# delehef/asgart

Hardware: AMD Instinct MI355X
Metric: Mbp/s probe+extend (direct+RC, k=20 g=100) (higher is better)
Workload: dtype u64 keys / u32 SA

## Files before the change

asgart_amd/csrc/device_base.hpp:

```cpp
#pragma once

#include "search_dev.hpp"

#include <type_traits>

namespace asgart {

constexpr int kTiers = 7;
constexpr int kRunsStat = kTiers + 1;

enum Counter {
    CT_BIG = 0,
    CT_SEG,
    CT_SCAN_TICKET,
    CT_FAM,
    CT_SD,
    CT_OVF,
    CT_TOTAL_HITS,
    CT_N_SKIPPED,
    CT_CARD_SKIPPED,
    CT_WITH_HITS,
    CT_RAW_HITS,
    CT_SEARCHED,
    CT_BISECT,
    CT_OVF_CURSOR,
    CT_AMBIG,
    CT_RANOUT,
    CT_EARLY_N = 34,
    CT_EARLY_CUR = 36,
    CT_RANK = 38,
    CT_BIG0 = 39,
    CT_ALG_BYTES = 68,
    CT_FLT_REJECTED,
    CT_LONGSEG,
    CT_ALG_BYTES16,
    CT_HIST_PEAK = 72,
    CT_HIST_PROBES = 88,
    CT_N1 = 104,
    CT_NF = 111,
    CT_CUR1 = 112,
    CT_CURF = 119,
    CT_OVF1 = 120,
    CT_BUSY1 = 128,
    CT_WGS1 = 136,
    CT_TPROBES1 = 144,
    CT_THITS1 = 152,
    CT_SEGMAX1 = 160,
    CT_CLUSTER_BARREN = 168,
    CT_CLUSTER_CUR = 169,
    CT_COUNT = 176
};

__device__ inline int chunk_of(const ChunkTable &ch, uint32_t g) {
    int lo = 0, hi = ch.n_chunks;
    while (hi - lo > 1) {
        int mid = (lo + hi) >> 1;
        if (ch.pbase[mid] <= g) lo = mid; else hi = mid;
    }
    return lo;
}

__device__ inline int chunk_of_uniform(const ChunkTable &ch, uint32_t g) {
    g = __builtin_amdgcn_readfirstlane(g);
    int lo = 0, hi = ch.n_chunks;
    while (hi - lo > 1) {
        const int mid = __builtin_amdgcn_readfirstlane((lo + hi) >> 1);
        if (ch.pbase[mid] <= g) lo = mid; else hi = mid;
    }
    return __builtin_amdgcn_readfirstlane(lo);
}

__device__ inline bool keep_hit(uint64_t x, uint64_t i, uint64_t s, uint64_t L, bool reverse) {
    if (!reverse) return x > i + s;
    return x != i && x >= s + L - i;
}

__device__ inline void lds_barrier() { __asm__ volatile("s_waitcnt lgkmcnt(0)\n\ts_barrier" ::: "memory"); }

__device__ inline uint32_t uni(uint32_t v) { return (uint32_t)__builtin_amdgcn_readfirstlane((int)v); }
__device__ inline unsigned long long uni(unsigned long long v) {
    return ((unsigned long long)uni((uint32_t)(v >> 32)) << 32) | uni((uint32_t)v);
}
__device__ inline uint32_t lane_of(uint32_t v, uint32_t l) {
    return (uint32_t)__builtin_amdgcn_readlane((int)v, (int)l);
}
__device__ inline unsigned long long lane_of(unsigned long long v, uint32_t l) {
    return ((unsigned long long)lane_of((uint32_t)(v >> 32), l) << 32) | lane_of((uint32_t)v, l);
}

__device__ inline uint32_t wave_incl_scan(uint32_t x) {
#define ASGART_DPP_ADD(ctrl, rows) \
    x += (uint32_t)__builtin_amdgcn_update_dpp(0, (int)x, ctrl, rows, 0xf, false)
    ASGART_DPP_ADD(0x111, 0xf);
    ASGART_DPP_ADD(0x112, 0xf);
    ASGART_DPP_ADD(0x114, 0xf);
    ASGART_DPP_ADD(0x118, 0xf);
    ASGART_DPP_ADD(0x142, 0xa);
    ASGART_DPP_ADD(0x143, 0xc);
#undef ASGART_DPP_ADD
    return x;
}

// ... 15 lines not shown
```

asgart_amd/csrc/extend_common_dev.hpp:

```cpp
#pragma once

#include "device_base.hpp"

namespace asgart {

constexpr uint32_t kTombstone = 0xFFFFFFFFu;

#ifdef ASGART_PROFILE_EXTEND
#define PROF_DECL unsigned long long pf_t0 = 0, pf_acc[12] = {0, 0, 0, 0, 0, 0, 0, 0, 0, 0, 0, 0}
#define PROF_START() pf_t0 = __builtin_amdgcn_s_memtime()
#define PROF_STOP(slot) pf_acc[slot] += __builtin_amdgcn_s_memtime() - pf_t0
#define PROF_COUNT(slot, v) pf_acc[slot] += (v)
#define PROF_MAX(slot, v) pf_acc[slot] = pf_acc[slot] > (unsigned long long)(v) ? pf_acc[slot] : (unsigned long long)(v)
#define PROF_SEG_BEGIN() const unsigned long long pf_seg0 = __builtin_amdgcn_s_memtime()
#define PROF_FLUSH()                                                             \
    do {                                                                         \
        const unsigned long long pf_dt = __builtin_amdgcn_s_memtime() - pf_seg0; \
        if (lane == 0 && atomicMax(&P.ctr[28], pf_dt) < pf_dt) {                 \
            P.ctr[29] = g0;                                                      \
            P.ctr[30] = ((unsigned long long)pf_acc[5] << 32) | pf_acc[3];       \
            P.ctr[31] = ((unsigned long long)pf_acc[10] << 32) | pf_acc[11];     \
            P.ctr[32] = pf_acc[0];                                               \
            P.ctr[33] = pf_acc[6];                                               \
            P.ctr[25] = pf_acc[9];                                               \
// ... 22 lines not shown
#define PROF_MAX(slot, v)
#define PROF_SEG_BEGIN()
#define PROF_FLUSH()
#endif
constexpr int kHitBatch = 1024;
constexpr uint32_t kNoSeq = 0xFFFFFFFFu;

struct RangeRun {
    uint32_t g_begin, g_stop;
    uint32_t g_seg0;
    uint32_t emit_from;
    uint32_t flags;
    uint32_t split;
    uint32_t pad0, pad1;
};
constexpr uint32_t kRunNoEmit = 1u;
constexpr uint32_t kRunLast = 2u;
constexpr uint32_t kRunDumpCap = 5120;
template <class PosT> constexpr uint32_t kDumpWords = sizeof(PosT) == 4 ? 8u : 12u;
struct SplitSeg {
    uint32_t g_seg0, run_base, n_ranges, cut_base;
    uint32_t span, hits, tier, warm;
};

template <class PosT>
struct ExtParams {
    const RangeRun *runs;
    uint32_t *run_meta, *run_dump;
    RunParams rp;
    const uint32_t *p_filt;
    const unsigned long long *row_off;
    const PosT *hits;
    const uint32_t *seg_list;
    const unsigned long long *n_seg_ptr;
    unsigned long long *cursor;
    SdRec *recs;
    unsigned long long rec_cap;
    uint32_t *ovf_list;
    unsigned long long *ovf_count;
    char *scratch;
    uint32_t gen_bits;
    uint32_t escalate_cost;
    uint32_t cap_limit;
    uint32_t heavy_cap;
    uint32_t solo_hits;
    uint32_t k8_delay;
    uint32_t tier;
    unsigned long long *seg_slots;
    unsigned long long *ctr;
    unsigned long long *hb;
};

template <class PosT>
__device__ inline void heartbeat(const ExtParams<PosT> &P, uint32_t g0, uint32_t at) {
    if (P.hb) {
        unsigned long long *slot = P.hb + 2u * (blockIdx.x % 256u);
        __builtin_nontemporal_store((unsigned long long)g0 | 1ull << 63, slot);
        __builtin_nontemporal_store((unsigned long long)at, slot + 1);
    }
}

template <class PosT>
__device__ inline bool arm_accepts(PosT x, PosT re, uint32_t thr, uint32_t k) {
    const PosT lo = (PosT)(re - k + 1u);
    const uint64_t w = thr ? (uint64_t)thr + k - 1u : 0u;
    return (uint64_t)(PosT)(x - lo) < w;
}

__device__ inline uint32_t arm_threshold(uint64_t left_len, uint32_t G) {
    const uint64_t tenth = left_len <= 0xFFFFFFFFull ? (uint64_t)((uint32_t)left_len / 10u) : left_len / 10u;
    const uint64_t thr = tenth > (uint64_t)G ? tenth : (uint64_t)G;
    return thr > 0xFFFFFFFFull ? 0xFFFFFFFFu : (uint32_t)thr;
}

constexpr uint32_t kRecChunk = 32;
constexpr uint32_t kVoidStart = 0xFFFFFFFFu;
struct RecAlloc {
    unsigned long long next = 0;
    uint32_t left = 0;
};
template <class PosT>
__device__ inline void wg_begin(const ExtParams<PosT> &P) {
    if (threadIdx.x == 0 && P.tier >= 1u && P.tier <= (uint32_t)kRunsStat) {
        atomicAdd(&P.ctr[CT_BUSY1 + P.tier - 1u], 0ull - wall_clock64());
    }
}
template <class PosT>
__device__ inline void seg_clock(const ExtParams<PosT> &P, bool last = false) {
    if (!P.seg_slots || P.tier < 2u || P.tier > (uint32_t)kRunsStat) return;
    const unsigned long long now = wall_clock64();
    const unsigned long long prev = atomicExch(&P.seg_slots[blockIdx.x & 4095u], last ? 0ull : now);
    if (prev && now > prev) atomicMax(&P.ctr[CT_SEGMAX1 + P.tier - 1u], now - prev);
}
template <class PosT>
__device__ inline void wg_busy(const ExtParams<PosT> &P) {
    if (threadIdx.x == 0 && P.tier >= 1u && P.tier <= (uint32_t)kRunsStat) {
        seg_clock(P, true);
        atomicAdd(&P.ctr[CT_BUSY1 + P.tier - 1u], wall_clock64());
        atomicAdd(&P.ctr[CT_WGS1 + P.tier - 1u], 1ull);
    }
}
template <class PosT>
__device__ inline void rec_flush(RecAlloc &ra, const ExtParams<PosT> &P, int lane) {
    if ((uint32_t)lane < ra.left && ra.next + (unsigned)lane < P.rec_cap) P.recs[ra.next + (unsigned)lane].g_start = kVoidStart;
    ra.left = 0;
}
template <class PosT>
__device__ inline unsigned long long rec_slot(RecAlloc &ra, const ExtParams<PosT> &P, unsigned long long em, int lane) {
    const uint32_t n = (uint32_t)__popcll(em);
    if (n > ra.left) {
        rec_flush(ra, P, lane);
        const uint32_t take = n > kRecChunk ? n : kRecChunk;
        unsigned long long b = 0;
        if (lane == 0) b = atomicAdd(&P.ctr[CT_SD], (unsigned long long)take);
        ra.next = lane_of(b, 0u);
        ra.left = take;
    }
    const unsigned long long at = ra.next + (unsigned)__popcll(em & ((1ull << lane) - 1ull));
    ra.next += n;
    ra.left -= n;
    return at;
}

struct SegHeader {
    uint64_t cs, cl;
    bool rev;
    uint32_t pb;
    uint32_t chunk_end;
    uint32_t g_end;
};
__device__ inline SegHeader load_segment(const RunParams &rp, uint32_t g0) {
    const int c = chunk_of_uniform(rp.ch, g0);
    SegHeader s;
    s.cs = rp.ch.start[c];
    s.cl = rp.ch.len[c];
    s.rev = (rp.mode_of(c) & 2u) != 0u;
    s.pb = rp.ch.pbase[c];
    s.chunk_end = rp.ch.pbase[c + 1];
    s.g_end = min(s.chunk_end, rp.win_end(g0));
    return s;
}

struct ProbeBatch {
    uint32_t f_l, rel_l;
    unsigned long long base;
    uint32_t n;
    uint32_t tot;
    unsigned long long hm, qm;
};
template <int HB>
// ... 73 lines not shown
```

asgart_amd/csrc/extend_k8_dev.hpp:

```cpp
#pragma once

#include "extend_fast_dev.hpp"

namespace asgart {

#ifdef ASGART_PROFILE_EXTEND
#define K7T_DECL unsigned long long k7t[4] = {0, 0, 0, 0}, k7t0 = 0, k7n = 0
#define K7T_MARK() k7t0 = __builtin_amdgcn_s_memtime()
#define K7T_LAP(j)                                                   \
    do {                                                             \
        const unsigned long long k7now = __builtin_amdgcn_s_memtime(); \
        k7t[j] += k7now - k7t0;                                      \
        k7t0 = k7now;                                                \
    } while (0)
#define K7T_STEP() ++k7n
#define K7C(slot, v) do { if (wave == 0u && lane == 0) atomicAdd(&P.ctr[slot], (unsigned long long)(v)); } while (0)
#define K7U_DECL unsigned long long k7u[8] = {0, 0, 0, 0, 0, 0, 0, 0}, k7u0 = 0
#define K7U_MARK() k7u0 = __builtin_amdgcn_s_memtime()
#define K7U_LAP(j)                                                   \
    do {                                                             \
        const unsigned long long k7now = __builtin_amdgcn_s_memtime(); \
        k7u[j] += k7now - k7u0;                                      \
        k7u0 = k7now;                                                \
    } while (0)
#define K7U_FLUSH()                                                                       \
    do {                                                                                  \
        if (lane == 0)                                                                    \
            for (int k7j = 0; k7j < 8; ++k7j) atomicAdd(&P.ctr[57 + k7j], k7u[k7j]);       \
        for (int k7j = 0; k7j < 8; ++k7j) k7u[k7j] = 0;                                   \
    } while (0)
#define K7T_FLUSH(cls)                                                                      \
    do {                                                                                    \
        if (lane == 0)                                                                      \
            for (int k7j = 0; k7j < 4; ++k7j) atomicAdd(&P.ctr[40 + 4 * (cls) + k7j], k7t[k7j]); \
        if (lane == 0 && (cls) == 0) atomicAdd(&P.ctr[52], k7n);                            \
        k7t[0] = k7t[1] = k7t[2] = k7t[3] = 0;                                              \
        k7n = 0;                                                                            \
    } while (0)
#else
#define K7T_DECL
#define K7T_MARK()
#define K7T_LAP(j)
#define K7T_STEP()
#define K7C(slot, v)
#define K7U_DECL
#define K7U_MARK()
#define K7U_LAP(j)
#define K7U_FLUSH()
#define K7T_FLUSH(cls)
#endif

#define K7_RARE(x) __builtin_expect(!!(x), 0)
#define K7_USUAL(x) __builtin_expect(!!(x), 1)

constexpr uint32_t K7_PREV = 1u;
constexpr uint32_t K7_CUR = 2u;
constexpr uint32_t K7_LATE = 4u;
constexpr uint32_t K7_LAST = 8u;
constexpr uint32_t K7_GIVEUP = 16u;
constexpr uint32_t K7_OVF = 1u;
constexpr uint32_t K7_STAGE = 2u;
constexpr uint32_t K7_CLEAR = 4u;


constexpr uint32_t K8_CLEARNOW = 32u;
constexpr uint32_t K8_OVF = 1u;
constexpr uint32_t K8_STILL = 2u;
constexpr uint32_t K8_BIG = 4u;

template <class PosT, int S, int NT, int HB, int kRows = 1024, int kE = 2, bool RANGE = false>
__global__ __launch_bounds__(NT) void extend_k8_kernel(ExtParams<PosT> P) {
    constexpr int NW = NT / 64, NWA = NW - 2;
    constexpr int CAP = S * NWA * 64;
    constexpr int NE = S * NWA;
    constexpr uint32_t kRowsWalk = 62;
    constexpr uint32_t kBitWords = (uint32_t)kRows / 32u;
    using Tab = ArmTable<PosT>;
    using WinT = typename Tab::WinT;
    constexpr bool kWidePos = Tab::kWidePos;
    constexpr uint32_t kTabBytes = (uint32_t)(kRows * kE * 8);
    constexpr uint32_t kCmdWords = 32;
    constexpr uint32_t kNewMax = kWidePos ? (uint32_t)HB / 2u : (uint32_t)HB;
    static_assert(!RANGE || S * NWA * 64 <= (int)kRunDumpCap, "runs over ranges: dump capacity");
    static_assert(NW >= 4 && HB <= 1024 && S <= 8 && NE <= 128 && (kRows & (kRows - 1)) == 0 && kE == 2 && kRows <= 2048 && CAP < 65536,
                  "shape");
    if (NT >= 1024) __builtin_amdgcn_s_setprio(3);

    __shared__ __attribute__((aligned(16))) unsigned long long s_tab[2][kRows * kE];
    __shared__ PosT s_hits[3 * HB];
    __shared__ __attribute__((aligned(16))) uint32_t s_best[3][HB];
    __shared__ unsigned long long s_stash[3][kStash];
    __shared__ uint32_t s_rowbits[3][kRows / 32];
    __shared__ __attribute__((aligned(16))) uint32_t s_pull[2][8];
    __shared__ uint32_t s_slot[2][NWA][8];
    __shared__ __attribute__((aligned(16))) uint32_t s_nstash[4];
#ifdef K8_SINGLE_FREE
    constexpr uint32_t kFreeBufs = 1;
#else
    constexpr uint32_t kFreeBufs = 2;
#endif
    __shared__ __attribute__((aligned(16))) uint32_t s_free[kFreeBufs][NWA][8];
    __shared__ PosT s_newx[2][kNewMax];
    __shared__ uint32_t s_newch[2][kNewMax];
    __shared__ uint16_t s_newh[2][RANGE ? kNewMax : 1u];
    __shared__ __attribute__((aligned(16))) uint32_t s_cmd[3][kCmdWords];
    __shared__ __attribute__((aligned(16))) uint32_t s_mid[8];
    __shared__ PosT s_cle[CAP], s_crs[CAP];
    __shared__ unsigned long long s_seg[3];
    __shared__ uint32_t s_end[4];
    __shared__ unsigned long long s_bcast;
    __shared__ uint32_t s_sink[64];
    __shared__ uint32_t s_never;

    const int tid = threadIdx.x, lane = tid & 63;
    const uint32_t wave = (uint32_t)__builtin_amdgcn_readfirstlane(tid >> 6);
    const bool is_rank = wave == (uint32_t)NWA, is_plan = wave == (uint32_t)(NWA + 1);
    const unsigned long long lt_mask = (1ull << lane) - 1ull;
    RecAlloc rec_alloc;
    wg_begin(P);
    K7T_DECL;
    K7U_DECL;
#ifdef ASGART_PROFILE_EXTEND
    unsigned long long k7_sum_a = 0, k7_sum_cnt = 0, k7_sum_n = 0;
#endif

    PosT a_ls[S], a_re[S];
    uint32_t a_thr[S], a_gap[S], a_seq[S], c_h[S];
#pragma unroll
    for (int L = 0; L < S; ++L) {
        a_seq[L] = kNoSeq;
        a_ls[L] = a_re[L] = 0;
        a_thr[L] = a_gap[L] = 0;
        c_h[L] = 0;
    }
    uint32_t livemask = 0;
    uint32_t gen = 0, par = 0, tri = 0;
    auto clear_table = [&]() {
        for (uint32_t e = tid; e < (uint32_t)(2 * kRows * kE); e += NT) (&s_tab[0][0])[e] = 0ull;
    };
    clear_table();
    if (tid == 0) s_never = kNever;
    lds_barrier();

    char *const tab0 = reinterpret_cast<char *>(&s_tab[0][0]);
    char *const best0 = reinterpret_cast<char *>(&s_best[0][0]);

    for (;;) {
        if (tid == 0) s_bcast = atomicAdd(P.cursor, 1ull);
        if (tid < 4) s_nstash[tid] = 0u;
        if (tid < 16) (&s_pull[0][0])[tid] = 0u;
        for (uint32_t j = tid; j < 3u * kBitWords; j += NT) (&s_rowbits[0][0])[j] = 0u;
        for (uint32_t j = tid; j < kFreeBufs * (uint32_t)(NWA * 8); j += NT) (&s_free[0][0][0])[j] = 64u;
        for (uint32_t j = tid; j < (uint32_t)(2 * NWA * 8); j += NT) (&s_slot[0][0][0])[j] = 0u;
        lds_barrier();
        const unsigned long long seg = uni(s_bcast);
        lds_barrier();
        if (seg >= *P.n_seg_ptr) break;
        RangeRun run{};
        uint32_t emit_from_i = 0;
        if constexpr (RANGE) {
            run = P.runs[seg];
            run.g_begin = uni(run.g_begin);
            run.g_stop = uni(run.g_stop);
            run.g_seg0 = uni(run.g_seg0);
            run.emit_from = uni(run.emit_from);
// ... 701 lines not shown
                atomicAdd(&P.ctr[26], k7_sum_a);
                atomicAdd(&P.ctr[27], k7_sum_cnt);
                atomicAdd(&P.ctr[21], k7_sum_n);
                const unsigned long long k7_dt = __builtin_amdgcn_s_memtime() - k7_seg0;
                if (atomicMax(&P.ctr[28], k7_dt) < k7_dt) {
                    P.ctr[29] = g0;
                    P.ctr[30] = k7_sum_n << 32;
                    P.ctr[31] = (k7_sum_a << 32) | (k7_sum_cnt & 0xffffffffull);
                }
            }
            k7_sum_a = k7_sum_cnt = k7_sum_n = 0;
#endif
            if (!overflow) {
                const uint32_t (*const fr)[8] = s_free[sp & (kFreeBufs - 1u)];
                const uint32_t fv = lane < NE ? fr[lane % NWA][lane / NWA] : 0u;
                uint32_t total_free = lane_of(wave_incl_scan(fv), 63u);
                if constexpr (NE > 64) {
                    const uint32_t fv2 = lane + 64 < NE ? fr[(lane + 64) % NWA][(lane + 64) / NWA] : 0u;
                    total_free += lane_of(wave_incl_scan(fv2), 63u);
                }
                const bool ran_out = uni(s_end[1]) != 0u;
                if constexpr (RANGE) {
                    if (lane == 0) {
                        uint32_t *m = P.run_meta + seg * 16ull;
                        m[1] = fam_seq;
                        m[2] = fam_open ? 1u : 0u;
                        m[3] = 0u;
                        m[5] = (uint32_t)wall_clock64() - s_end[3];
                    }
                }
                if (fam_open && total_free == (uint32_t)CAP) fam_open = false;
                if (RANGE && !(run.flags & kRunLast)) {
                } else if (ran_out) {
                    if (lane == 0) atomicAdd(&P.ctr[CT_RANOUT], 1ull);
                } else if (fam_open) {
                    emit_records(lane == 0, (PosT)0, (PosT)0, (PosT)0, (PosT)0, kTombstone, fam_seq);
                }
            } else if (lane == 0) {
                if constexpr (RANGE) {
                    P.run_meta[seg * 16ull + 4ull] = 1u;
                } else {
                    const unsigned long long at = atomicAdd(P.ovf_count, 1ull);
                    if (P.ovf_list) P.ovf_list[at] = g0;
                }
            }
        } else {
            const RunParams &rp = P.rp;
            const uint32_t k = (uint32_t)rp.k, step = (uint32_t)rp.step, G = rp.G;
            const uint32_t thr0 = arm_threshold(k, G);
            const uint32_t bsh = bucket_shift(G, k);
            const uint32_t kGenBits = min(Tab::kGenMax, max(2u, P.gen_bits));
            const uint32_t g0 = RANGE ? run.g_seg0 : P.seg_list[seg];
            if (lane == 0) {
                heartbeat(P, g0, 0u);
                seg_clock(P);
            }
            const SegHeader sg = load_segment(rp, g0);
            const uint32_t g_end = RANGE ? min(sg.g_end, run.g_stop) : sg.g_end;
            if (lane == 0) {
                if constexpr (RANGE) s_end[3] = (uint32_t)wall_clock64();
                s_seg[0] = g0;
                s_seg[1] = sg.cs;
                s_seg[2] = sg.cl | ((unsigned long long)sg.rev << 63);
            }
            uint32_t quiet = 0, pend = 0;
            bool done = false, giveup = false;
            uint32_t hbuf = 2;
            uint32_t g = RANGE ? run.g_begin : g0, pos = 0;
            ProbeBatch bt{};
            bool staged = false;
            auto open_batch = [&]() {
                if (lane == 0) heartbeat(P, g0, g);
                bt = load_batch<HB>(P.p_filt, P.row_off, g, g_end, lane);
                pos = 0;
                staged = false;
                return bt.n != 0u;
            };
            struct Probe {
                uint32_t cnt, off, tb, bb, g10, pend;
                uint64_t i;
            };
            struct Plan {
                uint32_t flags, pre;
                unsigned long long st_base;
                uint32_t st_tot, st_buf;
                Probe q;
            };
            const Probe no_probe{0, 0, 0, 0, 0, 0, 0};
            bool opened = false;
            auto next_probe = [&](Probe &nx) -> bool {
                for (;;) {
                    uint32_t q;
                    const uint32_t b = next_hit(bt, pos, q);
                    if (q) {
                        quiet += q;
                        pend += q * step;
                        if (quiet >= rp.tstar) {
                            done = true;
                            return false;
                        }
                    }
                    if (b < 64u) {
                        quiet = 0;
                        pos = b + 1;
                        opened = false;
                        if (!staged) {
                            hbuf = hbuf == 2u ? 0u : hbuf + 1u;
                            opened = true;
                            staged = true;
                        }
                        nx.cnt = lane_of(bt.f_l, b);
                        nx.off = hbuf * (uint32_t)HB + lane_of(bt.rel_l, b);
                        nx.i = (uint64_t)(g + b - sg.pb + 1) * step;
                        nx.pend = pend;
                        pend = 0;
                        return true;
                    }
                    g += bt.n;
                    if (g >= g_end) return false;
                    if (!open_batch()) {
                        giveup = true;
                        return false;
                    }
                }
            };
// ... 117 lines not shown
            for (uint32_t sc = 0, sp = 0;; sc = sc == 2u ? 0u : sc + 1u, sp ^= 1u) {
                const uint32_t sn = sc == 2u ? 0u : sc + 1u;
                const uint32_t cw = s_cmd[lane < 32 ? sc : sn][lane & 31];
                const uint32_t pflags_prev = s_pull[sp ^ 1u][0];
                const uint32_t pn_prev = s_pull[sp ^ 1u][1], pseq_prev = s_pull[sp ^ 1u][2];
                K7T_MARK();
                auto C = [&](int j) { return (uint32_t)__builtin_amdgcn_readlane((int)cw, j); };
                auto N = [&](int j) { return (uint32_t)__builtin_amdgcn_readlane((int)cw, 32 + j); };
                const uint32_t flags = C(0);
                if ((flags & K7_GIVEUP) || (uni(pflags_prev) & K8_OVF)) {
                    overflow = true;
                    break;
                }
                const bool more = !(flags & K7_LAST);
                const uint32_t nflags = more ? N(0) : 0u;
                if (uni(pflags_prev) & K8_BIG) {
                    big_rounds(Cur{k, pv_g10, bsh, pv_tabo, C(15), C(23), C(11), C(14)}, uni(pn_prev), uni(pseq_prev), thr0, sp ^ 1u);
                    lds_barrier();
                }
                if (flags & K8_CLEARNOW) clear_table();
                const uint32_t npre = more ? N(10) : 0u;
                const unsigned long long st_base = ((unsigned long long)N(25) << 32) | N(24);
                const uint32_t st_tot = N(26), st_buf = N(27);
                if (npre & K7_STAGE) fetch_rows(st_base, st_tot);
                if (more && (nflags & K7_CUR) && indexes(N(1)))
                    insert_hits(N(1), N(2), N(3), N(4), N(9), N(5), bsh, (nflags & K7_LATE) != 0u, st_base + (N(2) - st_buf * (uint32_t)HB));
                if (more && !(nflags & (K7_LAST | K7_GIVEUP))) {
                    const Plan p_after = advance(nflags);
                    write_cmd(sc == 0u ? 2u : sc - 1u, p_after, Before{N(1), N(6), N(7), N(2), N(9)});
                    if ((p_after.flags & K7_LAST) && lane == 0) {
                        s_end[1] = (!done && g_end < sg.chunk_end && (!RANGE || sg.g_end == g_end)) ? 1u : 0u;
                    }
                }
                if (npre & K7_STAGE) store_rows(st_tot, st_buf);
                pv_tabo = C(3);
                pv_g10 = C(5);
                K7T_LAP(0);
                lds_barrier();
                K7T_LAP(1);
                if (!more) break;
            }
#ifndef K8_TRACE_WAVE
            K7T_FLUSH(2);
#endif
            (void)thr0;
            (void)G;
        }
#pragma unroll
        for (int L = 0; L < S; ++L) a_seq[L] = kNoSeq;
        livemask = 0;
        lds_barrier();
    }
    rec_flush(rec_alloc, P, lane);
    wg_busy(P);
}

}
```

asgart_amd/csrc/pipeline.hip:

```cpp
#include "pipeline_dev.hpp"
#include "extend_wave_dev.hpp"
#include "extend_heavy_dev.hpp"
#include "extend_fast_dev.hpp"
#include "extend_k8_dev.hpp"

#include <algorithm>
#include <atomic>
#include <chrono>
#include <string>
#include <thread>

namespace asgart {

#ifdef ASGART_PROFILE_EXTEND
#define PROF_DUMP(tag)                                                                          \
    do {                                                                                       \
        fprintf(stderr, "[extend profile %s] stage=%llu batches=%llu | reg_cyc=%llu reg_probes=%llu | build=%llu "\
                "lds_probes=%llu match=%llu apply=%llu retire=%llu segs=%llu sumA=%llu sumCnt=%llu | longest: "   \
                "cyc=%llu g0=%llu lds_probes=%llu reg_probes=%llu sumA=%llu sumCnt=%llu stage=%llu match=%llu\n", \
                tag, h_ctr[16], h_ctr[17], h_ctr[18], h_ctr[19], h_ctr[20], h_ctr[21], h_ctr[22], h_ctr[23],  \
                h_ctr[24], h_ctr[25], h_ctr[26], h_ctr[27], h_ctr[28], h_ctr[29], h_ctr[30] >> 32,            \
                h_ctr[30] & 0xffffffffull, h_ctr[31] >> 32, h_ctr[31] & 0xffffffffull, h_ctr[32], h_ctr[33]); \
        fprintf(stderr, "    K7 steps=%llu; cycles [to barrier 1, wait, to barrier 2, wait]: control %llu %llu %llu %llu | arm wave 0 %llu %llu %llu %llu | last arm wave %llu %llu %llu %llu\n", \
                h_ctr[52], h_ctr[40], h_ctr[41], h_ctr[42], h_ctr[43], h_ctr[44], h_ctr[45], h_ctr[46], h_ctr[47], h_ctr[48], h_ctr[49], h_ctr[50], h_ctr[51]); \
// ... 696 lines not shown
        scratch7 = scratch6 + region;
        return 0;
    }

    void launch_kernel(int tier, uint64_t n_items, hipStream_t st) {
        ep.tier = (uint32_t)tier;
        ep.seg_slots = w.seg_slots.as<unsigned long long>() + (size_t)4096 * (size_t)(tier & 7);
        ep.hb = cx.d_hb ? cx.d_hb + (size_t)2 * SearchCtx::kHbSlots * (size_t)(tier & 7) : nullptr;
        auto grid = [&](uint64_t dflt) -> unsigned {
            uint64_t g = dflt;
            if (opt.grid[tier] > 0) g = tier >= 3 ? std::min<uint64_t>(dflt, (uint64_t)opt.grid[tier]) : (uint64_t)opt.grid[tier];
            return (unsigned)std::min<uint64_t>(n_items, g);
        };
        switch (tier) {
        case 1:
            extend_kernel<SlotT, kArmCapSmall><<<grid(kGrid1), 64, 0, st>>>(ep);
            break;
        case 2:
            if (arms_kernel)
                extend_fast_kernel<SlotT, kWaveArmsLayers<SlotT>, 64, kWaveArmsHits, 256, 2><<<grid(kGrid2Arms), 64, 0, st>>>(ep);
            else
                extend_heavy_kernel<SlotT, kArmCapMid, kMidThreads, 0><<<grid(kGrid2), kMidThreads, 0, st>>>(ep);
            break;
        case 3:
            extend_k8_kernel<SlotT, kK8LongLayers<SlotT>, 1024, kHitBatch, kFastLongRows<SlotT>, 2><<<grid(256), 1024, 0, st>>>(ep);
            break;
        case 4:
            if (arms_kernel)
                extend_fast_kernel<SlotT, kMidArmsLayers<SlotT>, 256, kWaveArmsHits, 512, 2><<<grid(256 * 4), 256, 0, st>>>(ep);
            else if constexpr (sizeof(SlotT) == 4)
                extend_heavy_kernel<SlotT, kArmCapBig32, kHeavyThreads, 0><<<grid(256), kHeavyThreads, 0, st>>>(ep);
            else
                extend_heavy_kernel<SlotT, kArmCapBig64, kHeavyThreads, 0><<<grid(256), kHeavyThreads, 0, st>>>(ep);
            break;
        case 5:
            extend_fast_kernel<SlotT, kMidArmsLayers<SlotT>, 512, kHitBatch, 1024, 2><<<grid(256 * 2), 512, 0, st>>>(ep);
            break;
        case 6:
            if (scratch_override) ep.scratch = scratch_override;
            if (arms_kernel)
                extend_fast_kernel<SlotT, kFastHeavyLayers<SlotT>, 1024, kHitBatch, kFastLongRows<SlotT>, 2><<<grid(256), 1024, 0, st>>>(ep);
            else
                extend_heavy_kernel<SlotT, caph, kHeavyThreads, 1><<<grid(256), kHeavyThreads, 0, st>>>(ep);
            ep.scratch = scratch6;
            break;
        default:
            ep.scratch = scratch_override ? scratch_override : scratch7;
            extend_heavy_kernel<SlotT, 1, kHeavyThreads, 2><<<grid(n_wg7), kHeavyThreads, 0, st>>>(ep);
            ep.scratch = scratch6;
            break;
        }
    }

    void launch_runs(uint32_t n_items) {
        ep.runs = reinterpret_cast<const RangeRun *>(d_split + kOffRuns);
        ep.run_meta = reinterpret_cast<uint32_t *>(d_split + kOffMeta);
        ep.run_dump = w.split_dump.as<uint32_t>();
        ep.seg_list = nullptr;
        ep.n_seg_ptr = reinterpret_cast<const unsigned long long *>(d_split);
        ep.cursor = reinterpret_cast<unsigned long long *>(d_split + 24);
        ep.ovf_list = nullptr;
        ep.ovf_count = d_ctr + CT_OVF1 + 2;
        ep.tier = kRunsStat;
        ep.seg_slots = w.seg_slots.as<unsigned long long>();
        ep.hb = cx.d_hb ? cx.d_hb : nullptr;
        extend_k8_kernel<SlotT, kK8LongLayers<SlotT>, 1024, kHitBatch, kFastLongRows<SlotT>, 2, true><<<n_items, 1024, 0, s>>>(ep);
    }

    void launch_tier(int tier) {
        if (tier < 1 || tier > kTiers || !n_t[tier - 1]) return;
        ep.seg_list = order + seg_off[tier - 1];
        ep.n_seg_ptr = d_ctr + CT_N1 + (tier - 1);
        ep.cursor = d_ctr + CT_CUR1 + (tier - 1);
        ep.ovf_list = tier < kTiers ? ovf[tier - 1] : nullptr;
        ep.ovf_count = d_ctr + CT_OVF1 + (tier - 1);
        launch_kernel(tier, n_t[tier - 1], tier_stream[tier]);
    #ifdef ASGART_PROFILE_EXTEND
        char tag[8];
        snprintf(tag, sizeof tag, "%d", tier);
        PROF_TIER(tag, tier_stream[tier], n_t[tier - 1]);
    #endif
    }

    int32_t run_tiers(int attempt) {
        RC_TRY(w.fam_sds.reserve((size_t)rec_cap * sizeof(SdRec)));
        HIP_TRY(hipMemsetAsync(d_ctr + CT_SD, 0, 8, s));
        HIP_TRY(hipMemsetAsync(d_ctr + CT_NF, 0, (size_t)(CT_COUNT - CT_NF) * 8, s));
        HIP_TRY(hipMemsetAsync(d_ctr + CT_EARLY_N, 0, 4 * 8, s));
        HIP_TRY(hipMemsetAsync(d_ctr + CT_BUSY1, 0, (size_t)(CT_COUNT - CT_BUSY1) * 8, s));
        RC_TRY(w.seg_slots.reserve((size_t)8 * 4096 * 8));
        HIP_TRY(hipMemsetAsync(w.seg_slots.p, 0, (size_t)8 * 4096 * 8, s));
        HIP_TRY(hipEventRecord(cx.ev[7], s));
        ep.rp = rp;
        ep.p_filt = p_filt;
        ep.row_off = row_off;
        ep.hits = hits;
        ep.recs = w.fam_sds.as<SdRec>();
        ep.rec_cap = rec_cap;
        ep.scratch = scratch6;
        ep.cap_limit = opt.test_cap_limit >= 0 ? (uint32_t)opt.test_cap_limit : 0xFFFFFFFFu;
        ep.escalate_cost = 0xFFFFFFFFu;
        ep.heavy_cap = (uint32_t)heavy_cap64;
        ep.solo_hits = opt.solo == 1 ? 16u : (uint32_t)opt.solo;
        ep.gen_bits = (uint32_t)opt.test_genbits;
        ep.k8_delay = (uint32_t)opt.test_k8_delay;
        ep.ctr = d_ctr;
        ep.hb = nullptr;
        RC_TRY(cx.heartbeat(opt.watchdog_s > 0));
        if (cx.h_hb) memset(cx.h_hb, 0, (size_t)SearchCtx::kHbTiers * SearchCtx::kHbSlots * 16);
        double est[kTiers + 1];
        plan_estimates(est);
        int32_t stream_of[kTiers], launch_seq[kTiers];
        RC_TRY(tier_plan(cx.n_tier_st, n_t, opt.tier_order, est + 1, n_runs ? est[0] : 0.0, stream_of, launch_seq));
        bool used[SearchCtx::kMaxTierStreams] = {};
        tier_stream[0] = s;
        for (int t = 1; t <= kTiers; ++t) {
            tier_ran[t] = false;
            tier_stream[t] = stream_of[t - 1] > 0 ? cx.tier_st[stream_of[t - 1] - 1] : s;
            if (stream_of[t - 1] > 0) used[stream_of[t - 1] - 1] = true;
        }
        for (int i = 0; i < cx.n_tier_st; ++i)
            if (used[i]) HIP_TRY(hipStreamWaitEvent(cx.tier_st[i], cx.ev[7], 0));
        if (opt.debug) {
            fprintf(stderr, "[asgart] tier plan (%d tier streams; 0 = main stream behind %.1f ms of range runs):", cx.n_tier_st,
                    n_runs ? est[0] : 0.0);
            for (int i = 0; i < kTiers && launch_seq[i]; ++i)
                fprintf(stderr, " t%d@%d ~%.1f ms", launch_seq[i], stream_of[launch_seq[i] - 1], est[launch_seq[i]]);
            fprintf(stderr, "\n");
        }
        scratch_override = nullptr;
        if (n_runs) {
            RC_TRY(w.split_dump.reserve((size_t)(n_runs + n_splits) * 2 * kRunDumpCap * kDumpWords<SlotT> * 4));
            HIP_TRY(hipMemsetAsync(d_split + 24, 0, 8, s));
            HIP_TRY(hipMemsetAsync(d_split + kOffMeta, 0, (size_t)n_runs * 64, s));
            launch_runs(n_runs);
            HIP_TRY(hipGetLastError());
            HIP_TRY(hipEventRecord(cx.runs_ev, s));
        }
        t_launch = std::chrono::steady_clock::now();
        for (int i = 0; i < kTiers && launch_seq[i]; ++i) {
            const int t = launch_seq[i];
            launch_tier(t);
            HIP_TRY(hipEventRecord(cx.tier_ev[t - 1], tier_stream[t]));
            tier_ran[t] = true;
        }
        HIP_TRY(hipGetLastError());
        if (cx.progress && attempt == 0) {
            if (!progress_given) {
                RC_TRY(wd_event_sync(idx, cx, cx.ev[3], "the hit rows"));
                signal_progress();
            }
        }
        for (int t = 0; t <= kTiers; ++t) early_n[t] = 0;
        {
            struct Early {
                int src, dst;
                hipEvent_t ev;
                hipStream_t st;
                bool pending;
            } early[2] = {{3, 0, cx.tier_ev[2], tier_stream[3], false}, {6, 0, cx.tier_ev[5], tier_stream[6], false}};
            int n_pending = 0;
            unsigned early_polls = 0;
            Watchdog early_wd(idx, cx);
            for (int e = 0; e < 2; ++e) {
                Early &E = early[e];
                int dst = E.src + 1;
                while (dst < kTiers && (!tier_enabled(dst) || tier_cap[dst] <= tier_cap[E.src])) ++dst;
                E.dst = dst;
                E.pending = n_t[E.src - 1] && E.st != s && (dst < kTiers || !n_t[kTiers - 1]);
                n_pending += E.pending ? 1 : 0;
            }
            if (early[0].pending && early[1].pending && early[0].dst == early[1].src) {
                early[0].pending = false;
                --n_pending;
            }
            while (n_pending) {
                bool progressed = false;
                for (int e = 0; e < 2; ++e) {
                    Early &E = early[e];
                    if (!E.pending) continue;
                    const hipError_t q = hipEventQuery(E.ev);
                    if (q == hipErrorNotReady) {
                        (void)hipGetLastError();
                        continue;
                    }
                    HIP_TRY(q);
                    E.pending = false;
                    --n_pending;
                    progressed = true;
                    HIP_TRY(hipMemcpyAsync(h_scalar + 1 + e, d_ctr + CT_OVF1 + E.src - 1, 8, hipMemcpyDeviceToHost, s));
// ... 1007 lines not shown
```

Before: 43760.

## Fuse range-run extension and tier-3 segments into one joint kernel launch

Adds a joint kernel that hands out workgroup tickets through an atomic counter. The first n_runs tickets run the range-run extension body and the rest run the tier-3 segment body. Shared memory moves to templated namespace-scope arrays so both bodies can share one kernel. The goal is to fill GPU idle time while the range runs drain and to save a separate tier-3 launch on another stream, at the cost of changing the tier plan and scheduling behaviour.

Measured after the change: 46920, median of 6. 1.07x the previous value.

```diff
diff --git a/asgart_amd/csrc/device_base.hpp b/asgart_amd/csrc/device_base.hpp
--- a/asgart_amd/csrc/device_base.hpp
+++ b/asgart_amd/csrc/device_base.hpp
@@ -48,6 +48,7 @@
     CT_SEGMAX1 = 160,
     CT_CLUSTER_BARREN = 168,
     CT_CLUSTER_CUR = 169,
+    CT_JOINT_TICKET = 171,
     CT_COUNT = 176
 };
 
diff --git a/asgart_amd/csrc/extend_common_dev.hpp b/asgart_amd/csrc/extend_common_dev.hpp
--- a/asgart_amd/csrc/extend_common_dev.hpp
+++ b/asgart_amd/csrc/extend_common_dev.hpp
@@ -98,9 +98,9 @@
 };
 
 template <class PosT>
-__device__ inline void heartbeat(const ExtParams<PosT> &P, uint32_t g0, uint32_t at) {
+__device__ inline void heartbeat(const ExtParams<PosT> &P, uint32_t g0, uint32_t at, uint32_t wg = blockIdx.x) {
     if (P.hb) {
-        unsigned long long *slot = P.hb + 2u * (blockIdx.x % 256u);
+        unsigned long long *slot = P.hb + 2u * (wg % 256u);
         __builtin_nontemporal_store((unsigned long long)g0 | 1ull << 63, slot);
         __builtin_nontemporal_store((unsigned long long)at, slot + 1);
     }
@@ -132,16 +132,16 @@
     }
 }
 template <class PosT>
-__device__ inline void seg_clock(const ExtParams<PosT> &P, bool last = false) {
+__device__ inline void seg_clock(const ExtParams<PosT> &P, bool last = false, uint32_t wg = blockIdx.x) {
     if (!P.seg_slots || P.tier < 2u || P.tier > (uint32_t)kRunsStat) return;
     const unsigned long long now = wall_clock64();
-    const unsigned long long prev = atomicExch(&P.seg_slots[blockIdx.x & 4095u], last ? 0ull : now);
+    const unsigned long long prev = atomicExch(&P.seg_slots[wg & 4095u], last ? 0ull : now);
     if (prev && now > prev) atomicMax(&P.ctr[CT_SEGMAX1 + P.tier - 1u], now - prev);
 }
 template <class PosT>
-__device__ inline void wg_busy(const ExtParams<PosT> &P) {
+__device__ inline void wg_busy(const ExtParams<PosT> &P, uint32_t wg = blockIdx.x) {
     if (threadIdx.x == 0 && P.tier >= 1u && P.tier <= (uint32_t)kRunsStat) {
-        seg_clock(P, true);
+        seg_clock(P, true, wg);
         atomicAdd(&P.ctr[CT_BUSY1 + P.tier - 1u], wall_clock64());
         atomicAdd(&P.ctr[CT_WGS1 + P.tier - 1u], 1ull);
     }
diff --git a/asgart_amd/csrc/extend_k8_dev.hpp b/asgart_amd/csrc/extend_k8_dev.hpp
--- a/asgart_amd/csrc/extend_k8_dev.hpp
+++ b/asgart_amd/csrc/extend_k8_dev.hpp
@@ -68,10 +68,48 @@
 constexpr uint32_t K8_STILL = 2u;
 constexpr uint32_t K8_BIG = 4u;
 
-template <class PosT, int S, int NT, int HB, int kRows = 1024, int kE = 2, bool RANGE = false>
-__global__ __launch_bounds__(NT) void extend_k8_kernel(ExtParams<PosT> P) {
-    constexpr int NW = NT / 64, NWA = NW - 2;
-    constexpr int CAP = S * NWA * 64;
+
+#define K8_SHAPE class PosT, int S, int NT, int HB, int kRows, int kE
+#define K8_SHAPE_ARGS PosT, S, NT, HB, kRows, kE
+template <K8_SHAPE>
+struct K8Shape {
+    static constexpr int NW = NT / 64, NWA = NW - 2;
+    static constexpr int CAP = S * NWA * 64;
+    static constexpr uint32_t kCmdWords = 32;
+    static constexpr uint32_t kNewMax = sizeof(PosT) == 8 ? (uint32_t)HB / 2u : (uint32_t)HB;
+#ifdef K8_SINGLE_FREE
+    static constexpr uint32_t kFreeBufs = 1;
+#else
+    static constexpr uint32_t kFreeBufs = 2;
+#endif
+};
+template <K8_SHAPE> __shared__ __attribute__((aligned(16))) unsigned long long k8_tab[2][kRows * kE];
+template <K8_SHAPE> __shared__ PosT k8_hits[3 * HB];
+template <K8_SHAPE> __shared__ __attribute__((aligned(16))) uint32_t k8_best[3][HB];
+template <K8_SHAPE> __shared__ unsigned long long k8_stash[3][kStash];
+template <K8_SHAPE> __shared__ uint32_t k8_rowbits[3][kRows / 32];
+template <K8_SHAPE> __shared__ __attribute__((aligned(16))) uint32_t k8_pull[2][8];
+template <K8_SHAPE> __shared__ uint32_t k8_slot[2][K8Shape<K8_SHAPE_ARGS>::NWA][8];
+template <K8_SHAPE> __shared__ __attribute__((aligned(16))) uint32_t k8_nstash[4];
+template <K8_SHAPE> __shared__ __attribute__((aligned(16))) uint32_t k8_free[K8Shape<K8_SHAPE_ARGS>::kFreeBufs][K8Shape<K8_SHAPE_ARGS>::NWA][8];
+template <K8_SHAPE> __shared__ PosT k8_newx[2][K8Shape<K8_SHAPE_ARGS>::kNewMax];
+template <K8_SHAPE> __shared__ uint32_t k8_newch[2][K8Shape<K8_SHAPE_ARGS>::kNewMax];
+template <K8_SHAPE> __shared__ uint16_t k8_newh[2][K8Shape<K8_SHAPE_ARGS>::kNewMax];
+template <K8_SHAPE> __shared__ __attribute__((aligned(16))) uint32_t k8_cmd[3][K8Shape<K8_SHAPE_ARGS>::kCmdWords];
+template <K8_SHAPE> __shared__ __attribute__((aligned(16))) uint32_t k8_mid[8];
+template <K8_SHAPE> __shared__ PosT k8_cle[K8Shape<K8_SHAPE_ARGS>::CAP];
+template <K8_SHAPE> __shared__ PosT k8_crs[K8Shape<K8_SHAPE_ARGS>::CAP];
+template <K8_SHAPE> __shared__ unsigned long long k8_seg[3];
+template <K8_SHAPE> __shared__ uint32_t k8_end[4];
+template <K8_SHAPE> __shared__ unsigned long long k8_bcast;
+template <K8_SHAPE> __shared__ uint32_t k8_sink[64];
+template <K8_SHAPE> __shared__ uint32_t k8_never;
+
+template <K8_SHAPE, bool RANGE>
+__device__ __forceinline__ void extend_k8_body(const ExtParams<PosT> &P, const uint32_t wg) {
+    using Sh = K8Shape<K8_SHAPE_ARGS>;
+    constexpr int NW = Sh::NW, NWA = Sh::NWA;
+    constexpr int CAP = Sh::CAP;
     constexpr int NE = S * NWA;
     constexpr uint32_t kRowsWalk = 62;
     constexpr uint32_t kBitWords = (uint32_t)kRows / 32u;
@@ -79,38 +117,34 @@
     using WinT = typename Tab::WinT;
     constexpr bool kWidePos = Tab::kWidePos;
     constexpr uint32_t kTabBytes = (uint32_t)(kRows * kE * 8);
-    constexpr uint32_t kCmdWords = 32;
-    constexpr uint32_t kNewMax = kWidePos ? (uint32_t)HB / 2u : (uint32_t)HB;
+    constexpr uint32_t kNewMax = Sh::kNewMax;
+    constexpr uint32_t kFreeBufs = Sh::kFreeBufs;
     static_assert(!RANGE || S * NWA * 64 <= (int)kRunDumpCap, "runs over ranges: dump capacity");
     static_assert(NW >= 4 && HB <= 1024 && S <= 8 && NE <= 128 && (kRows & (kRows - 1)) == 0 && kE == 2 && kRows <= 2048 && CAP < 65536,
                   "shape");
     if (NT >= 1024) __builtin_amdgcn_s_setprio(3);
 
-    __shared__ __attribute__((aligned(16))) unsigned long long s_tab[2][kRows * kE];
-    __shared__ PosT s_hits[3 * HB];
-    __shared__ __attribute__((aligned(16))) uint32_t s_best[3][HB];
-    __shared__ unsigned long long s_stash[3][kStash];
-    __shared__ uint32_t s_rowbits[3][kRows / 32];
-    __shared__ __attribute__((aligned(16))) uint32_t s_pull[2][8];
-    __shared__ uint32_t s_slot[2][NWA][8];
-    __shared__ __attribute__((aligned(16))) uint32_t s_nstash[4];
-#ifdef K8_SINGLE_FREE
-    constexpr uint32_t kFreeBufs = 1;
-#else
-    constexpr uint32_t kFreeBufs = 2;
-#endif
-    __shared__ __attribute__((aligned(16))) uint32_t s_free[kFreeBufs][NWA][8];
-    __shared__ PosT s_newx[2][kNewMax];
-    __shared__ uint32_t s_newch[2][kNewMax];
-    __shared__ uint16_t s_newh[2][RANGE ? kNewMax : 1u];
-    __shared__ __attribute__((aligned(16))) uint32_t s_cmd[3][kCmdWords];
-    __shared__ __attribute__((aligned(16))) uint32_t s_mid[8];
-    __shared__ PosT s_cle[CAP], s_crs[CAP];
-    __shared__ unsigned long long s_seg[3];
-    __shared__ uint32_t s_end[4];
-    __shared__ unsigned long long s_bcast;
-    __shared__ uint32_t s_sink[64];
-    __shared__ uint32_t s_never;
+    constexpr auto &s_tab = k8_tab<K8_SHAPE_ARGS>;
+    constexpr auto &s_hits = k8_hits<K8_SHAPE_ARGS>;
+    constexpr auto &s_best = k8_best<K8_SHAPE_ARGS>;
+    constexpr auto &s_stash = k8_stash<K8_SHAPE_ARGS>;
+    constexpr auto &s_rowbits = k8_rowbits<K8_SHAPE_ARGS>;
+    constexpr auto &s_pull = k8_pull<K8_SHAPE_ARGS>;
+    constexpr auto &s_slot = k8_slot<K8_SHAPE_ARGS>;
+    constexpr auto &s_nstash = k8_nstash<K8_SHAPE_ARGS>;
+    constexpr auto &s_free = k8_free<K8_SHAPE_ARGS>;
+    constexpr auto &s_newx = k8_newx<K8_SHAPE_ARGS>;
+    constexpr auto &s_newch = k8_newch<K8_SHAPE_ARGS>;
+    constexpr auto &s_newh = k8_newh<K8_SHAPE_ARGS>;
+    constexpr auto &s_cmd = k8_cmd<K8_SHAPE_ARGS>;
+    constexpr auto &s_mid = k8_mid<K8_SHAPE_ARGS>;
+    constexpr auto &s_cle = k8_cle<K8_SHAPE_ARGS>;
+    constexpr auto &s_crs = k8_crs<K8_SHAPE_ARGS>;
+    constexpr auto &s_seg = k8_seg<K8_SHAPE_ARGS>;
+    constexpr auto &s_end = k8_end<K8_SHAPE_ARGS>;
+    constexpr auto &s_bcast = k8_bcast<K8_SHAPE_ARGS>;
+    constexpr auto &s_sink = k8_sink<K8_SHAPE_ARGS>;
+    constexpr auto &s_never = k8_never<K8_SHAPE_ARGS>;
 
     const int tid = threadIdx.x, lane = tid & 63;
     const uint32_t wave = (uint32_t)__builtin_amdgcn_readfirstlane(tid >> 6);
@@ -918,8 +952,8 @@
             const uint32_t kGenBits = min(Tab::kGenMax, max(2u, P.gen_bits));
             const uint32_t g0 = RANGE ? run.g_seg0 : P.seg_list[seg];
             if (lane == 0) {
-                heartbeat(P, g0, 0u);
-                seg_clock(P);
+                heartbeat(P, g0, 0u, wg);
+                seg_clock(P, false, wg);
             }
             const SegHeader sg = load_segment(rp, g0);
             const uint32_t g_end = RANGE ? min(sg.g_end, run.g_stop) : sg.g_end;
@@ -936,7 +970,7 @@
             ProbeBatch bt{};
             bool staged = false;
             auto open_batch = [&]() {
-                if (lane == 0) heartbeat(P, g0, g);
+                if (lane == 0) heartbeat(P, g0, g, wg);
                 bt = load_batch<HB>(P.p_filt, P.row_off, g, g_end, lane);
                 pos = 0;
                 staged = false;
@@ -1160,7 +1194,27 @@
         lds_barrier();
     }
     rec_flush(rec_alloc, P, lane);
-    wg_busy(P);
+    wg_busy(P, wg);
 }
 
+template <class PosT, int S, int NT, int HB, int kRows = 1024, int kE = 2, bool RANGE = false>
+__global__ __launch_bounds__(NT) void extend_k8_kernel(ExtParams<PosT> P) {
+    extend_k8_body<K8_SHAPE_ARGS, RANGE>(P, blockIdx.x);
 }
+
+template <class PosT, int S, int NT, int HB, int kRows = 1024, int kE = 2>
+__global__ __launch_bounds__(NT) void extend_k8_joint_kernel(ExtParams<PosT> PR, ExtParams<PosT> PT, uint32_t n_run_wgs,
+                                                             unsigned long long *ticket) {
+    static_assert(2 * sizeof(ExtParams<PosT>) + 16 <= 4096, "kernel arguments: HIP passes at most 4 KB");
+    constexpr auto &s_bcast = k8_bcast<K8_SHAPE_ARGS>;
+    if (threadIdx.x == 0) s_bcast = atomicAdd(ticket, 1ull);
+    lds_barrier();
+    const uint32_t mine = (uint32_t)uni(s_bcast);
+    lds_barrier();
+    if (mine < n_run_wgs) extend_k8_body<K8_SHAPE_ARGS, true>(PR, mine);
+    else extend_k8_body<K8_SHAPE_ARGS, false>(PT, mine - n_run_wgs);
+}
+#undef K8_SHAPE
+#undef K8_SHAPE_ARGS
+
+}
diff --git a/asgart_amd/csrc/pipeline.hip b/asgart_amd/csrc/pipeline.hip
--- a/asgart_amd/csrc/pipeline.hip
+++ b/asgart_amd/csrc/pipeline.hip
@@ -772,7 +772,7 @@
         }
     }
 
-    void launch_runs(uint32_t n_items) {
+    void set_runs_params() {
         ep.runs = reinterpret_cast<const RangeRun *>(d_split + kOffRuns);
         ep.run_meta = reinterpret_cast<uint32_t *>(d_split + kOffMeta);
         ep.run_dump = w.split_dump.as<uint32_t>();
@@ -784,7 +784,30 @@
         ep.tier = kRunsStat;
         ep.seg_slots = w.seg_slots.as<unsigned long long>();
         ep.hb = cx.d_hb ? cx.d_hb : nullptr;
+    }
+    void launch_runs(uint32_t n_items) {
+        set_runs_params();
         extend_k8_kernel<SlotT, kK8LongLayers<SlotT>, 1024, kHitBatch, kFastLongRows<SlotT>, 2, true><<<n_items, 1024, 0, s>>>(ep);
+    }
+
+    void launch_runs_and_tier3(uint32_t n_items) {
+        ep.seg_list = order + seg_off[3 - 1];
+        ep.n_seg_ptr = d_ctr + CT_N1 + (3 - 1);
+        ep.cursor = d_ctr + CT_CUR1 + (3 - 1);
+        ep.ovf_list = ovf[3 - 1];
+        ep.ovf_count = d_ctr + CT_OVF1 + (3 - 1);
+        ep.tier = 3u;
+        ep.seg_slots = w.seg_slots.as<unsigned long long>() + (size_t)4096 * 3;
+        ep.hb = cx.d_hb ? cx.d_hb + (size_t)2 * SearchCtx::kHbSlots * 3 : nullptr;
+        const ExtParams<SlotT> ep3 = ep;
+        uint64_t grid3 = std::min<uint64_t>(n_t[3 - 1], 256);
+        if (opt.grid[3] > 0) grid3 = std::min<uint64_t>(grid3, (uint64_t)opt.grid[3]);
+        set_runs_params();
+        extend_k8_joint_kernel<SlotT, kK8LongLayers<SlotT>, 1024, kHitBatch, kFastLongRows<SlotT>, 2>
+            <<<n_items + (unsigned)grid3, 1024, 0, s>>>(ep, ep3, n_items, d_ctr + CT_JOINT_TICKET);
+        if (opt.debug)
+            fprintf(stderr, "[asgart] joint launch on the main stream: %u workgroups for the runs over ranges + %u for tier 3's %llu segment(s)\n",
+                    n_items, (unsigned)grid3, (unsigned long long)n_t[3 - 1]);
     }
 
     void launch_tier(int tier) {
@@ -808,6 +831,7 @@
         HIP_TRY(hipMemsetAsync(d_ctr + CT_NF, 0, (size_t)(CT_COUNT - CT_NF) * 8, s));
         HIP_TRY(hipMemsetAsync(d_ctr + CT_EARLY_N, 0, 4 * 8, s));
         HIP_TRY(hipMemsetAsync(d_ctr + CT_BUSY1, 0, (size_t)(CT_COUNT - CT_BUSY1) * 8, s));
+        static_assert(CT_JOINT_TICKET > CT_BUSY1 && CT_JOINT_TICKET < CT_COUNT, "the joint launch's tickets start from zero");
         RC_TRY(w.seg_slots.reserve((size_t)8 * 4096 * 8));
         HIP_TRY(hipMemsetAsync(w.seg_slots.p, 0, (size_t)8 * 4096 * 8, s));
         HIP_TRY(hipEventRecord(cx.ev[7], s));
@@ -831,7 +855,12 @@
         double est[kTiers + 1];
         plan_estimates(est);
         int32_t stream_of[kTiers], launch_seq[kTiers];
-        RC_TRY(tier_plan(cx.n_tier_st, n_t, opt.tier_order, est + 1, n_runs ? est[0] : 0.0, stream_of, launch_seq));
+        const bool joint = n_runs && n_t[3 - 1];
+        uint64_t n_plan[kTiers];
+        for (int t = 0; t < kTiers; ++t) n_plan[t] = n_t[t];
+        if (joint) n_plan[3 - 1] = 0;
+        const double main_ms = joint ? std::max(est[0], est[3]) : (n_runs ? est[0] : 0.0);
+        RC_TRY(tier_plan(cx.n_tier_st, n_plan, opt.tier_order, est + 1, main_ms, stream_of, launch_seq));
         bool used[SearchCtx::kMaxTierStreams] = {};
         tier_stream[0] = s;
         for (int t = 1; t <= kTiers; ++t) {
@@ -842,8 +871,8 @@
         for (int i = 0; i < cx.n_tier_st; ++i)
             if (used[i]) HIP_TRY(hipStreamWaitEvent(cx.tier_st[i], cx.ev[7], 0));
         if (opt.debug) {
-            fprintf(stderr, "[asgart] tier plan (%d tier streams; 0 = main stream behind %.1f ms of range runs):", cx.n_tier_st,
-                    n_runs ? est[0] : 0.0);
+            fprintf(stderr, "[asgart] tier plan (%d tier streams; 0 = main stream behind %.1f ms of range runs%s):", cx.n_tier_st,
+                    main_ms, joint ? " and tier 3, one launch" : "");
             for (int i = 0; i < kTiers && launch_seq[i]; ++i)
                 fprintf(stderr, " t%d@%d ~%.1f ms", launch_seq[i], stream_of[launch_seq[i] - 1], est[launch_seq[i]]);
             fprintf(stderr, "\n");
@@ -853,9 +882,14 @@
             RC_TRY(w.split_dump.reserve((size_t)(n_runs + n_splits) * 2 * kRunDumpCap * kDumpWords<SlotT> * 4));
             HIP_TRY(hipMemsetAsync(d_split + 24, 0, 8, s));
             HIP_TRY(hipMemsetAsync(d_split + kOffMeta, 0, (size_t)n_runs * 64, s));
-            launch_runs(n_runs);
+            if (joint) launch_runs_and_tier3(n_runs);
+            else launch_runs(n_runs);
             HIP_TRY(hipGetLastError());
             HIP_TRY(hipEventRecord(cx.runs_ev, s));
+            if (joint) {
+                HIP_TRY(hipEventRecord(cx.tier_ev[3 - 1], s));
+                tier_ran[3] = true;
+            }
         }
         t_launch = std::chrono::steady_clock::now();
         for (int i = 0; i < kTiers && launch_seq[i]; ++i) {
```
